# showlab/DiffSim

Hardware: AMD Instinct MI355X
Metric: image-pairs/sec at 512px, SD1.5 up_blocks[0] t=600 (higher is better)
Workload: dtype bf16

## Files before the change

### diffsim_amd/csrc/attention.hip

```cpp
#include "common.h"

#include <type_traits>

namespace dsim {
namespace {

__device__ __forceinline__ float max_halves(float x) {
    const unsigned u = __float_as_uint(x);
    const auto r = __builtin_amdgcn_permlane32_swap(u, u, false, false);
    return fmaxf(__uint_as_float(r[0]), __uint_as_float(r[1]));
}

constexpr int KT = 64;

template <typename T, int D> struct ACfg {
    static constexpr int ES = sizeof(T);
    static constexpr int VEC = 16 / ES;
    static constexpr int NKS = (D + 15) / 16;
    static constexpr int NDB = (D + 31) / 32;
    static constexpr int DPL = NDB * 32;
    static constexpr bool ONES = D < DPL;
    static constexpr int DPLK = (ES == 2) ? NKS * 16 : DPL;
    static constexpr int RS = DPLK * ES + 16;
    static constexpr bool KONE = (ES == 2) && (D % 16 == 8);
// ... 809 lines not shown
        if (__syncthreads_or(bad)) attend2<T, D, false>(qf, (const T*)p.k + kvoff, (const T*)p.v + kvoff, p.ldk, p.Nk, smem, oa, l);
    }
#pragma unroll
    for (int qb = 0; qb < 2; ++qb) {
        if (q[qb] >= p.Nq) continue;
        T* orow = (T*)p.out + ((size_t)b * p.Nq + q[qb]) * p.ldo + h * D;
        store_o_rows<D>(orow, half, wide_rows(p), [&](int db, int r) { return oa[qb].b[db][r]; });
    }
}

template <typename T, int D, bool FASTK>
__global__ __launch_bounds__(256, (ACfg<T, D>::WPS)) void attn_kernel(const AttnArgs p, const float scale_log2) {
    typedef ACfg<T, D> C;
    extern __shared__ __attribute__((aligned(16))) char smem[];
    const int lane = threadIdx.x & 63, wave = threadIdx.x >> 6, half = lane >> 5, l31 = lane & 31;
    const int nqb = (p.Nq + 127) / 128;
    int bid = blockIdx.x;
    if (p.xcd_remap) {
        const int nwg = gridDim.x, xcd = bid & 7, qq = nwg >> 3, r = nwg & 7, slot = bid >> 3;
        bid = (xcd < r ? xcd * (qq + 1) : r * (qq + 1) + (xcd - r) * qq) + slot;
    }
    const int qblk = bid % nqb, bh = bid / nqb;
    const int h = bh % p.H, b = bh / p.H;
    const int q = qblk * 128 + wave * 32 + l31;
    const int qc = q < p.Nq ? q : p.Nq - 1;
    const T* qrow = (const T*)p.q + ((size_t)b * p.Nq + qc) * p.ldq + h * D;
    QFrags<T, D> qf;
    load_q<T, D>(qf, qrow, half, scale_log2);
    const size_t kvoff = (size_t)(b % p.Bkv) * p.Nk * p.ldk + h * D;
    OAcc<T, D> oa;
    attend_checked<T, D, FASTK>(qf, (const T*)p.k + kvoff, (const T*)p.v + kvoff, p.ldk, p.Nk, smem, oa);
    auto& o = oa.b;
    if (q < p.Nq) {
        T* orow = (T*)p.out + ((size_t)b * p.Nq + q) * p.ldo + h * D;
        if constexpr (sizeof(T) == 2) {
            store_o_rows<D>((h16*)orow, half, wide_rows(p), [&](int db, int r) { return o[db][r]; });
        } else {
#pragma unroll
            for (int db = 0; db < C::NDB; ++db)
#pragma unroll
                for (int g = 0; g < 4; ++g) {
                    const int d = db * 32 + 8 * g + 4 * half;
                    if (d < D) {
                        f32x4 v4;
#pragma unroll
                        for (int j = 0; j < 4; ++j) v4[j] = o[db][4 * g + j];
                        *reinterpret_cast<f32x4*>(orow + d) = v4;
                    }
                }
        }
    }
}

template <int D, bool K80>
__global__ __launch_bounds__(256, 2) void attn_short_kernel(const AttnArgs p, const float scale_log2, const int qit) {
    typedef h16 T;
    typedef ACfg<T, D> C;
    constexpr int KR = 96;
    constexpr int CPRD = D / C::VEC;
    constexpr int VOFF = KR * C::RS;
    extern __shared__ __attribute__((aligned(16))) char smem[];
    const int tid = threadIdx.x, lane = tid & 63, wave = tid >> 6, half = lane >> 5, l31 = lane & 31;
    const int nqb = (p.Nq + 127) / 128;
    const int nbmax = (p.B + p.Bkv - 1) / p.Bkv;
    const int nch = (nbmax * nqb + qit - 1) / qit;
    int bid = blockIdx.x;
    if (p.xcd_remap) {
        const int nwg = gridDim.x, xcd = bid & 7, qq = nwg >> 3, r = nwg & 7, slot = bid >> 3;
        bid = (xcd < r ? xcd * (qq + 1) : r * (qq + 1) + (xcd - r) * qq) + slot;
    }
    const int h = bid % p.H, t0 = bid / p.H, ch = t0 % nch, bkv = t0 / nch;
    const int nbg = (p.B - bkv + p.Bkv - 1) / p.Bkv;
    if (ch * qit >= nbg * nqb) return;
    const size_t kvoff = (size_t)bkv * p.Nk * p.ldk + h * D;
    const T* kb = (const T*)p.k + kvoff;
    const T* vb = (const T*)p.v + kvoff;
    {
        const u32x4 z = {0u, 0u, 0u, 0u};
        for (int o = tid * 16; o < KR * (C::RS + C::RSV); o += 256 * 16) *reinterpret_cast<u32x4*>(smem + o) = z;
        __syncthreads();
        for (int idx = tid; idx < p.Nk * CPRD; idx += 256) {
            const int r = idx / CPRD, c = idx - r * CPRD;
            const u32x4 kk = *reinterpret_cast<const u32x4*>(kb + (size_t)r * p.ldk + c * C::VEC);
            const u32x4 vv = *reinterpret_cast<const u32x4*>(vb + (size_t)r * p.ldk + c * C::VEC);
            *reinterpret_cast<u32x4*>(smem + r * C::RS + c * 16) = kk;
            *reinterpret_cast<u32x4*>(smem + VOFF + r * C::RSV + c * 16) = vv;
        }
        if constexpr (C::ONES)
            for (int r = tid; r < p.Nk; r += 256) *reinterpret_cast<u32x4*>(smem + VOFF + r * C::RSV + CPRD * 16) = one_chunk<T>();
        __syncthreads();
    }
    const int i16 = lane & 15, g4 = lane >> 4;
    const char* const kfr = smem + l31 * C::RS + half * 16;
    const char* const vfr = smem + VOFF + (4 * (g4 >> 1) + (i16 >> 2)) * C::RSV + (16 * (g4 & 1) + 4 * (i16 & 3)) * 2;
    auto load_q_raw = [&](QFrags<T, D>& f, int b, int q) {
        const int qq = q < p.Nq ? q : p.Nq - 1;
        const T* qrow = (const T*)p.q + ((size_t)b * p.Nq + qq) * p.ldq + h * D;
#pragma unroll
        for (int ks = 0; ks < C::NKS; ++ks) {
            const int d0 = 16 * ks + 8 * half;
            if (d0 < D) f.f[ks] = *reinterpret_cast<const h16x8*>(qrow + d0);
            else zero_frag(f.f[ks]);
        }
    };
    float bias[8];
#pragma unroll
    for (int r = 0; r < 8; ++r) bias[r] = (64 + (r & 3) + 8 * (r >> 2) + 4 * half >= p.Nk) ? -INFINITY : 0.f;
    typedef float f32x2 __attribute__((ext_vector_type(2)));
    const f32x2 c2 = {scale_log2, scale_log2};
    const bool wide = wide_rows(p);

    int bi = (ch * qit) / nqb, qblk = ch * qit - bi * nqb;
    QFrags<T, D> qf;
    load_q_raw(qf, bi * p.Bkv + bkv, qblk * 128 + wave * 32 + l31);
    for (int it = 0; it < qit && bi < nbg; ++it) {
        const int b = bi * p.Bkv + bkv;
        const int q = qblk * 128 + wave * 32 + l31;
        if (++qblk == nqb) { qblk = 0; ++bi; }
        QFrags<T, D> qn;
        load_q_raw(qn, (bi < nbg ? bi : nbg - 1) * p.Bkv + bkv, qblk * 128 + wave * 32 + l31);
        if (q - l31 < p.Nq) {
            f32x16 s[3];
#pragma unroll
            for (int kbk = 0; kbk < 3; ++kbk) {
#pragma unroll
                for (int r = 0; r < 16; ++r) s[kbk][r] = 0.f;
#pragma unroll
                for (int ks = 0; ks < C::NKS; ++ks) {
                    h16x8 kf;
                    lload_frag(kf, kfr + kbk * 32 * C::RS + ks * 32);
                    mma(kf, qf.f[ks], s[kbk]);
                }
            }
            float m = -INFINITY;
#pragma unroll
            for (int kbk = 0; kbk < 3; ++kbk)
#pragma unroll
                for (int r = 0; r < ((K80 && kbk == 2) ? 8 : 16); ++r) {
                    if constexpr (!K80) {
                        const int kv = kbk * 32 + (r & 3) + 8 * (r >> 2) + 4 * half;
                        if (kv >= p.Nk) s[kbk][r] = -INFINITY;
                    } else if (kbk == 2) {
                        s[kbk][r] += bias[r];
                    }
                    m = fmaxf(m, s[kbk][r]);
                }
            m = max_halves(m);
            const float mc = -m * scale_log2;
            const f32x2 m2 = {mc, mc};
            float psum = 0.f;
#pragma unroll
            for (int kbk = 0; kbk < 3; ++kbk)
#pragma unroll
                for (int r = 0; r < ((K80 && kbk == 2) ? 8 : 16); r += 2) {
                    const f32x2 e = __builtin_elementwise_fma((f32x2){s[kbk][r], s[kbk][r + 1]}, c2, m2);
                    s[kbk][r] = __builtin_amdgcn_exp2f(e[0]);
                    s[kbk][r + 1] = __builtin_amdgcn_exp2f(e[1]);
                    if constexpr (!C::ONES) psum += s[kbk][r] + s[kbk][r + 1];
                }
            f32x16 o[C::NDB];
#pragma unroll
            for (int db = 0; db < C::NDB; ++db)
#pragma unroll
                for (int r = 0; r < 16; ++r) o[db][r] = 0.f;
#pragma unroll
            for (int kbk = 0; kbk < 3; ++kbk)
#pragma unroll
                for (int s2 = 0; s2 < ((K80 && kbk == 2) ? 1 : 2); ++s2) {
                    h16x8 pf;
#pragma unroll
                    for (int e = 0; e < 8; ++e) pf[e] = (h16)s[kbk][8 * s2 + e];
#pragma unroll
                    for (int db = 0; db < C::NDB; ++db) {
                        const char* pa = vfr + (kbk * 32 + 16 * s2) * C::RSV + db * 64;
                        const h16x4 lo = h16_ds_read_tr16_b64((pa));
                        const h16x4 hi = h16_ds_read_tr16_b64((pa + 8 * C::RSV));
                        h16x8 vf;
#pragma unroll
                        for (int e = 0; e < 4; ++e) { vf[e] = lo[e]; vf[4 + e] = hi[e]; }
                        o[db] = H16_MFMA_32x32x16(vf, pf, o[db], 0, 0, 0);
                    }
                }
            float l_tot;
            if constexpr (C::ONES) {
                constexpr int RB = D / 32, RR = D % 32;
                constexpr int RH = (RR >> 2) & 1, REG = (RR & 3) + 4 * (RR >> 3);
                const float mine = o[RB][REG];
                const float other = __shfl_xor(mine, 32);
                l_tot = (half == RH) ? mine : other;
            } else {
                l_tot = psum + __shfl_xor(psum, 32);
            }
            const float inv = 1.0f / l_tot;
            if (q < p.Nq) {
                T* orow = (T*)p.out + ((size_t)b * p.Nq + q) * p.ldo + h * D;
                store_o_rows<D>(orow, half, wide, [&](int db, int r) { return o[db][r] * inv; });
            }
        }
        qf = qn;
    }
}


template <typename T, int D, typename S, typename F>
__device__ __forceinline__ S fold_rounded(const OAcc<T, D>& acc, int half, S s, F&& f) {
    typedef float f32x2 __attribute__((ext_vector_type(2)));
#pragma unroll
    for (int db = 0; db < ACfg<T, D>::NDB; ++db)
#pragma unroll
        for (int r = 0; r < 16; r += 2) {
            T v[2];
            if constexpr (sizeof(T) == 2) {
                const h16x2 p = __builtin_convertvector((f32x2){acc.b[db][r], acc.b[db][r + 1]}, h16x2);
                v[0] = p[0]; v[1] = p[1];
            } else {
                v[0] = acc.b[db][r]; v[1] = acc.b[db][r + 1];
            }
#pragma unroll
            for (int e = 0; e < 2; ++e) {
                const int rr = r + e, d = db * 32 + (rr & 3) + 8 * (rr >> 2) + 4 * half;
                if (d < D) s = f(s, db, rr, d, v[e]);
            }
        }
    return s;
}

template <typename T, int D>
__device__ __forceinline__ void settle(OAcc<T, D>& acc) {
#pragma unroll
    for (int db = 0; db < ACfg<T, D>::NDB; ++db)
#pragma unroll
        for (int r = 0; r < 16; ++r) {
            if (db * 32 + (r & 3) + 8 * (r >> 2) >= D) continue;
            float x = acc.b[db][r];
            asm volatile("" : "+v"(x));
            acc.b[db][r] = x;
        }
}

struct TailSums { float s0 = 0.f, s1 = 0.f, s2 = 0.f; };
template <typename T, int D, typename Y>
__device__ __forceinline__ TailSums tail_products(const OAcc<T, D>& ox, int half, int mse, Y&& y) {
    return fold_rounded<T, D>(ox, half, TailSums{}, [&](TailSums s, int db, int r, int d, T xr) {
        const float x = (float)xr, yv = y(db, r, d);
        if (mse) { const float df = x - yv; s.s0 = fmaf(df, df, s.s0); }
        else { s.s0 = fmaf(x, yv, s.s0); s.s1 = fmaf(x, x, s.s1); s.s2 = fmaf(yv, yv, s.s2); }
        return s;
    });
}

__device__ __forceinline__ void store_block_partial(TailSums t, int lane, int wave, float* __restrict__ o) {
    __shared__ float red[4][4];
// ... 125 lines not shown
        set = (int)blockIdx.z >= p.n_a;
        iq = ix = (int)blockIdx.z - (set ? p.n_a : 0);
    } else {
        qtile = blockIdx.x % qt;
        const int cd = blockIdx.x / qt;
        cell = cd >> 1; dir = cd & 1;
        const int ia = cell / p.n_b, ib = cell - ia * p.n_b;
        set = dir;
        iq = dir ? ib : ia;
        ix = dir ? ia : ib;
    }
    const T* qg = (const T*)p.q[set];
    const T* kg = (const T*)p.k[set ^ (self_mode ? 0 : 1)];
    const T* vg = (const T*)p.v[set ^ (self_mode ? 0 : 1)];
    T* so = (T*)p.self[set] + iq * img + boff;
    const int q = qtile * 128 + wave * 32 + l31;
    const int qc = q < N ? q : N - 1;
    QFrags<T, D> qf;
    load_q<T, D>(qf, qg + iq * img + boff + (size_t)qc * ld, half, scale_log2);
    OAcc<T, D> oa;
    attend<T, D>(qf, kg + ix * img + boff, vg + ix * img + boff, ld, N, smem, oa);
    settle<T, D>(oa);
    if (self_mode) {
        if (q < N) fold_rounded<T, D>(oa, half, 0, [&](int, int, int, int d, T y) { so[(size_t)q * ld + d] = y; return 0; });
        return;
    }
    TailSums t;
    if (q < N) t = tail_products<T, D>(oa, half, mse, [&](int, int, int d) { return (float)so[(size_t)q * ld + d]; });
    store_block_partial(t, lane, wave, part + ((((size_t)cell * 2 + dir) * gridDim.y + bh) * qt + qtile) * 4);
}

inline float scale_log2_of(int D) { return (1.0f / sqrtf((float)D)) * 1.4426950408889634f; }


constexpr int ATTN_FAST_MIN = 1024;

AttnKernel attention_kernel(const AttnArgs& a, int dtype) {
    if (dtype == DSIM_F32) return AttnKernel::Exact;
    if (sdpa160_applies(a)) return AttnKernel::P160;
    if ((a.D == 40 || a.D == 64 || a.D == 80 || a.D == 160) && a.Nk <= 96)
        return a.Nk > 64 && a.Nk <= 80 ? AttnKernel::ShortK80 : AttnKernel::Short;
    if (a.D == 40 && a.Nk >= 2048 && a.Nk % KT == 0) return AttnKernel::Long;
    if (a.D == 64 && a.Nk > 96 && a.Nq >= 256) return a.Nk >= ATTN_FAST_MIN ? AttnKernel::Q2Fast : AttnKernel::Q2;
    return a.Nk >= ATTN_FAST_MIN ? AttnKernel::Fast : AttnKernel::Exact;
}

template <typename T, int D>
int launch_attn_d(const AttnArgs& a, AttnKernel kind, hipStream_t s) {
    typedef ACfg<T, D> C;
    switch (kind) {
        case AttnKernel::Short:
        case AttnKernel::ShortK80:
            if constexpr (sizeof(T) == 2 && (D == 40 || D == 64 || D == 80 || D == 160)) {
                constexpr int LDSK = 96 * (C::RS + C::RSV);
                constexpr int LDSS = LDSK < 56 * 1024 ? 56 * 1024 : LDSK;
                const int nqb = (a.Nq + 127) / 128, nvb = ((a.B + a.Bkv - 1) / a.Bkv) * nqb;
                const long want = (D > 80 ? 2L : 8L) * cu_count();
                int qit = 8;
                while (qit > 1 && (long)((nvb + qit - 1) / qit) * a.H * a.Bkv < want) qit >>= 1;
                const int nch = (nvb + qit - 1) / qit;
                const dim3 g(nch * a.H * a.Bkv);
                if (kind == AttnKernel::ShortK80) {
                    static DeviceOnce onces;
                    auto kern = attn_short_kernel<D, true>;
                    CK_ONCE(onces, kern, LDSS);
                    hipLaunchKernelGGL(kern, g, dim3(256), LDSS, s, a, scale_log2_of(D), qit);
                    g_attn_last_launch = AttnLaunchRec{DSIM_ATTN_SHORT_K80, D, DSIM_H16, 1, qit, (int)g.x};
                } else {
                    static DeviceOnce onces;
                    auto kern = attn_short_kernel<D, false>;
                    CK_ONCE(onces, kern, LDSS);
                    hipLaunchKernelGGL(kern, g, dim3(256), LDSS, s, a, scale_log2_of(D), qit);
                    g_attn_last_launch = AttnLaunchRec{DSIM_ATTN_SHORT, D, DSIM_H16, 0, qit, (int)g.x};
                }
                DSIM_HIP_CHECK(hipGetLastError());
                return DSIM_OK;
            }
            break;
        case AttnKernel::Long:
            if constexpr (sizeof(T) == 2 && D == 40) {
                constexpr int LDS3 = 3 * 2 * C::TILE;
#ifdef DSIM_DEVTOOLS
                switch (g_attn_dbg) {
#define X(d) case d: { static DeviceOnce o; auto k = attn_long_kernel<D, d>; CK_ONCE(o, k, LDS3); hipLaunchKernelGGL(k, dim3(((a.Nq + 255) / 256) * a.H * a.B), dim3(256), LDS3, s, a, scale_log2_of(D)); DSIM_HIP_CHECK(hipGetLastError()); return DSIM_OK; }
                    X(8) X(32) X(64) X(96)
#undef X
                    default: break;
                }
#endif
                static DeviceOnce once2;
                auto kern = attn_long_kernel<D, 0>;
                CK_ONCE(once2, kern, LDS3);
                const dim3 gl(((a.Nq + 255) / 256) * a.H * a.B);
                hipLaunchKernelGGL(kern, gl, dim3(256), LDS3, s, a, scale_log2_of(D));
                g_attn_last_launch = AttnLaunchRec{DSIM_ATTN_LONG, D, DSIM_H16, 0, 0, (int)gl.x};
                DSIM_HIP_CHECK(hipGetLastError());
                return DSIM_OK;
            }
            break;
        case AttnKernel::Q2:
        case AttnKernel::Q2Fast:
            if constexpr (sizeof(T) == 2 && D == 64) {
                const dim3 grid2(((a.Nq + 255) / 256) * a.H * a.B);
                if (kind == AttnKernel::Q2Fast) {
                    static DeviceOnce o1;
                    auto k = attn_q2_kernel<D, true>;
                    CK_ONCE(o1, k, C::LDS);
                    hipLaunchKernelGGL(k, grid2, dim3(256), C::LDS, s, a, scale_log2_of(D));
                    g_attn_last_launch = AttnLaunchRec{DSIM_ATTN_Q2FAST, D, DSIM_H16, 0, 0, (int)grid2.x};
                } else {
                    static DeviceOnce o2;
                    auto k = attn_q2_kernel<D, false>;
                    CK_ONCE(o2, k, C::LDS);
                    hipLaunchKernelGGL(k, grid2, dim3(256), C::LDS, s, a, scale_log2_of(D));
// ... 129 lines not shown
            }
        }
        red[1][t] = x2t; red[2][t] = y2t;
        __syncthreads();
        for (int s = NT / 2; s > 0; s >>= 1) {
            if (t < s) { red[1][t] += red[1][t + s]; red[2][t] += red[2][t + s]; }
            __syncthreads();
        }
        const double den = mse ? (double)BH * N * D : fmax(sqrt(red[1][0]), 1e-8) * fmax(sqrt(red[2][0]), 1e-8);
        double ct = 0.0;
        for (int i = t; i < N; i += NT) {
            const double c = fold(0, i) / den;
            ct += c;
            if (co) co[i] = (float)c;
        }
        __syncthreads();
        red[0][t] = ct;
        __syncthreads();
        for (int s = NT / 2; s > 0; s >>= 1) {
            if (t < s) red[0][t] += red[0][t + s];
            __syncthreads();
        }
        res += red[0][0];
        __syncthreads();
    }
    if (t == 0) {
        const float sc = (float)(res * 0.5);
        score[p] = sc;
        if (status) status[p] = (sc - sc == 0.0f) ? 0 : 1;
    }
}

template <typename T>
int launch_maps_t(const void* q, const void* k, const void* v, const int32_t* ia, const int32_t* ib, int n_pairs, int B, int H, int N,
                  int D, int mse, float* score, float* local, float* contrib, int32_t* status, void* scratch, hipStream_t s) {
    return with_head_dim(D, [&](auto dc) -> int {
        constexpr int Dc = decltype(dc)::value, LDS = ACfg<T, Dc>::LDS;
        static DeviceOnce once;
        auto kern = pair_map_kernel<T, Dc>;
        CK_ONCE(once, kern, LDS);
        hipLaunchKernelGGL(kern, dim3((N + 127) / 128, B * H, n_pairs * 2), dim3(256), LDS, s, (const T*)q, (const T*)k, (const T*)v, ia,
                           ib, B, H, N, scale_log2_of(Dc), mse, (float*)scratch);
        hipLaunchKernelGGL(pair_map_finish_kernel, dim3(n_pairs), dim3(MAP_FINISH_THREADS), 0, s, (const float*)scratch, B * H, N, Dc,
                           mse, score, local, contrib, status);
        DSIM_HIP_CHECK(hipGetLastError());
        return DSIM_OK;
    });
}

}

#ifdef DSIM_DEVTOOLS
int g_attn_dbg = 0;
#endif

inline namespace DSIM_H16_NS {
const char* attention_kernel_kind(const AttnArgs& a, int dtype) { return attn_kind_suffix((int)attention_kernel(a, dtype)); }

static bool attention_args_ok(const AttnArgs& a, int dtype) {
    const int vec = dtype == DSIM_F32 ? 4 : 8;
    return !(a.D % 8 || a.ldq % vec || a.ldk % vec || a.ldo % 4 || a.Nk < 1 || a.Nq < 1 || a.Bkv < 1);
}

int attention_plan(const AttnArgs& a, int dtype) {
    if (!attention_args_ok(a, dtype)) return DSIM_ERR_INVALID;
    bool own = dtype == DSIM_H16;
#ifndef DSIM_H16_IS_F16
    own |= dtype == DSIM_F32;
    if (dtype == DSIM_F16) return DSIM_F16_TWIN(attention_plan(a, dtype));
#endif
    if (!own) return DSIM_ERR_INVALID;
    const int st = with_head_dim(a.D, [](auto) { return DSIM_OK; });
    return st != DSIM_OK ? st : (int)attention_kernel(a, dtype);
}

int launch_attention(const AttnArgs& a, int dtype, hipStream_t s) {
    if (!attention_args_ok(a, dtype)) return DSIM_ERR_INVALID;
    if (dtype == DSIM_H16) {
        const AttnKernel kind = attention_kernel(a, dtype);
        return kind == AttnKernel::P160 ? launch_sdpa160(a, s) : launch_attn_t<h16>(a, kind, s);
    }
#ifndef DSIM_H16_IS_F16
    if (dtype == DSIM_F32) return launch_attn_t<float>(a, attention_kernel(a, dtype), s);
    if (dtype == DSIM_F16) return DSIM_F16_TWIN(launch_attention(a, dtype, s));
#endif
    return DSIM_ERR_INVALID;
}

size_t pair_score_scratch_bytes(int n_pairs, int B, int H, int N, int D) {
    const size_t tiled = (size_t)n_pairs * 2 * B * H * ((N + 127) / 128) * 4 * sizeof(float);
    if (pair_score160_applies(N, D, DSIM_H16)) {
        const size_t pers = pair_score160_scratch_bytes(n_pairs, B, H);
        return pers > tiled ? pers : tiled;
    }
    return tiled;
}

int launch_pair_score(const void* q, const void* k, const void* v, const int32_t* ia, const int32_t* ib,
                      int n_pairs, int B, int H, int N, int D, int dtype, int similarity, float* out, void* scratch,
                      size_t scratch_bytes, hipStream_t s, int32_t* status) {
    if (n_pairs <= 0 || D % 8 || N < 1) return DSIM_ERR_INVALID;
    if (scratch_bytes < pair_score_scratch_bytes(n_pairs, B, H, N, D)) return DSIM_ERR_WORKSPACE;
    if (n_pairs * 2 > 65535) return DSIM_ERR_INVALID;
    if (dtype == DSIM_H16) {
        if (pair_score160_applies(N, D, DSIM_H16))
            return launch_pair_score160(q, k, v, ia, ib, n_pairs, B, H, similarity, out, scratch, scratch_bytes, s, status);
// ... 67 lines not shown
```

### diffsim_amd/csrc/common.h

```cpp
#pragma once
#include <hip/hip_runtime.h>
#include <stddef.h>
#include <stdint.h>

#include "../../include/diffsim_amd.h"

namespace dsim {

typedef __bf16 bf16_t;
typedef _Float16 f16_t;
#ifdef DSIM_H16_IS_F16
typedef _Float16 h16;
#define DSIM_H16_NS f16
#define DSIM_H16 DSIM_F16
#define DSIM_H16_ONE_BITS 0x3C00u
#define DSIM_H16_LSUM_MAX 3.0e4f
#define H16_MFMA_16x16x32 __builtin_amdgcn_mfma_f32_16x16x32_f16
#define H16_MFMA_32x32x16 __builtin_amdgcn_mfma_f32_32x32x16_f16
#else
typedef __bf16 h16;
#define DSIM_H16_NS bf16
#define DSIM_H16 DSIM_BF16
#define DSIM_H16_ONE_BITS 0x3F80u
#define DSIM_H16_LSUM_MAX 1e30f
// ... 34 lines not shown

enum GemmMode { GEMM_LINEAR = 0, GEMM_CONV3 = 1, GEMM_CONV3P = 2 };
enum GemmEpi { EPI_NONE = 0, EPI_RESIDUAL = 1, EPI_GEGLU = 2 };

struct GemmArgs {
    const void* A0 = nullptr;
    const void* A1 = nullptr;
    int C0 = 0, C1 = 0;
    int mode = GEMM_LINEAR;
    int Hin = 0, Win = 0, Hout = 0, Wout = 0;
    int stride = 1, ups = 0;
    int pad = 1;
    int lwo = -1, lhw = -1;
    int M = 0, N = 0, K = 0;
    const void* W = nullptr;
    const float* bias = nullptr;
    const float* bias2 = nullptr;
    int rows_per_batch = 0;
    int act = 0;
    const float* gate = nullptr;
    const float* gate2 = nullptr;
    int epi = EPI_NONE;
    int geglu_blk = 32;
    const void* residual = nullptr;
    void* out = nullptr;
    int ldo = 0;
    int out_split = 0;
    long long out_split_stride = 0;
    int force_big = 0;
    int wb_rows = 0;
    unsigned wb_stride = 0;
    float* gn_part = nullptr;
    int gn_hw = 0;
    const void* zero_page = nullptr;
    unsigned a0_bytes = 0, a1_bytes = 0, w_bytes = 0, out_bytes = 0;
#ifdef DSIM_DEVTOOLS
    int exp = 0;
    unsigned long long* stamps = nullptr;
#endif
};
struct GemmLaunchRec {
    int bm = 0, bn = 0, mode = -1, geglu = 0, ek = -1, small = 0;
};
extern thread_local GemmLaunchRec g_gemm_last_launch;
inline int geglu_block_rows(int N) { return (N % 320 == 0 && N != 8 * 320) ? 16 : 32; }
#ifdef DSIM_DEVTOOLS
extern int g_gemm_persistent;
extern int g_force_bm;
extern int g_gemm_exp;
extern int g_gemm_skinny;
extern unsigned long long* g_gemm_stamps;
extern int g_skinny_tile;
extern int g_attn_dbg;
extern float* g_tail160_dbg;
extern int g_tail160_exp;
extern int g_ff_dbg;
extern int g_rl_dbg;
extern int g_rl_wpc;
extern int g_ff_stagger;
#else
constexpr int g_gemm_skinny = 1, g_gemm_persistent = 1, g_force_bm = 0;
#endif
int pack_linear(const void* src, int src_dtype, void* dst, int dst_dtype, int N, int K,
                int geglu_interleave, hipStream_t s);
int pack_conv3(const void* src, int src_dtype, void* dst, int dst_dtype, int Cout, int Cin,
               hipStream_t s);
int pack_conv_in(const void* src, int src_dtype, float* dst, int Cout, int Cin, hipStream_t s);
int pack_vector(const void* src, int src_dtype, float* dst, int N, int geglu_interleave,
                hipStream_t s);
int gemv_f32(const void* W, int w_dtype, const void* bias, int b_dtype, const float* x, float* y,
             int N, int K, int act, hipStream_t s);
int add_vectors_f32(const float* a, const float* b, float* out, int N, hipStream_t s);
int timestep_sincos(float* out, int dim, int t, hipStream_t s);
int sincos_values(float* out, int dim, const float* vals , int count, hipStream_t s);

int prep_conv_in(const float* lat, const float* noise , float sa, float sb, const float* w ,
                 const float* bias, void* out, int dtype, int n_img, int Cin, int S, int Cout, int dup ,
                 hipStream_t st);
bool conv_in_rows_applies(int Cin, int S, int Cout);
int conv_in_rows(const float* images, const float* w , const float* bias, void* out, int dtype, int n_img, int S,
                 float* gn_part, hipStream_t st);
int convert_f32_to(const float* src, void* dst, int dtype, size_t n, hipStream_t s);
int gather_ctx(const float* ctx, int n_ctx, const int32_t* index, void* dst, int dtype, int n_images, size_t per, hipStream_t s);
int dup_batch(const void* in, void* out, int n_batch, size_t bytes_per_elem, hipStream_t s);
int resize_nearest(const void* in, void* out, int B, int Hin, int Win, int Hout, int Wout, size_t row_bytes, hipStream_t s);

struct RowLinArgs {
    const void* x = nullptr;
    void* out = nullptr;
    const float* ln_g = nullptr;
    const float* ln_b = nullptr;
    const void* stream = nullptr;
    int M = 0, C = 0, N = 0;
    float eps = 1e-5f;
    int dtype = DSIM_BF16;
};

int image_preprocess(const unsigned char* hwc, float* out, int n, int H, int W, int half, hipStream_t s);
int latent_sample(const float* moments, const float* eps, float* out, int n_out, int first, int stride, int C, int hw, int eps_n,
                  float sf, int round16, hipStream_t s);

size_t groupnorm_scratch_bytes(int B, int groups);
int groupnorm_passes(int C0, int C1, int HW, int groups, int dtype);
int groupnorm_plan(int C0, int C1, int B, int HW, int groups, int dtype, int pre, dsim_gn_plan* plan);
int layernorm_plan(int M, int C, int dtype, int mod, dsim_ln_plan* plan);
int launch_groupnorm(const void* x0, int C0, const void* x1, int C1, const float* gamma,
// ... 102 lines not shown
```

### diffsim_amd/csrc/rowres.hip

```cpp
#include "common.h"

namespace dsim {
namespace {

constexpr int RC = 320;
constexpr int RKS = RC / 16;
constexpr int RNB = RC / 32;
constexpr int RNCH = 4 * RC / 32;
constexpr int RITER = RNCH + 2;
constexpr int RW1B = 64 * RC * 2;
constexpr int RW2B = RC * 64;
constexpr int RCHB = RW1B + RW2B;
constexpr int RPIECES = RCHB / 1024;
constexpr int RPW = RPIECES / 4;
constexpr int RB1 = 0, RB2 = 8 * RC, RLG = 9 * RC, RLB = 10 * RC, RVEC = 11 * RC;
constexpr int RSCR = 32 * 144;
constexpr int RLDS = 2 * RCHB + RVEC * 4 + 4 * RSCR;
static_assert(RPIECES % 4 == 0 && RITER % 2 == 0, "ring geometry");

__global__ void pack_ff_stream_kernel(const h16* __restrict__ w1p, const h16* __restrict__ w2p, char* __restrict__ stream) {
    const int i = blockIdx.x * blockDim.x + threadIdx.x;
    if (i >= RITER * (RCHB / 16)) return;
    const int ci = i / (RCHB / 16), o = (i - ci * (RCHB / 16)) * 16;
    u32x4 v = {0u, 0u, 0u, 0u};
// ... 20 lines not shown
}

struct FFParams {
    const h16* x;
    h16* out;
    const float* ln_g;
    const float* ln_b;
    const char* stream;
    const float* b1;
    const float* b2;
    int M;
    float eps;
    unsigned x_bytes, stream_bytes;
    int stagger;
};

template <int DBG>
__global__ __launch_bounds__(256, 1) void ff_fused_kernel(const FFParams p, const int ntiles) {
    extern __shared__ __attribute__((aligned(16))) char smem[];
    const int tid = threadIdx.x, lane = tid & 63, l31 = lane & 31, half = lane >> 5;
    const int wave = __builtin_amdgcn_readfirstlane(tid >> 6);
    constexpr unsigned OOB = 0x80000000u;

    const __amdgpu_buffer_rsrc_t rX = __builtin_amdgcn_make_buffer_rsrc((void*)p.x, 0, (int)p.x_bytes, 0x00020000);
    const __amdgpu_buffer_rsrc_t rO = __builtin_amdgcn_make_buffer_rsrc((void*)p.out, 0, (int)p.x_bytes, 0x00020000);
    const __amdgpu_buffer_rsrc_t rS = __builtin_amdgcn_make_buffer_rsrc((void*)p.stream, 0, (int)p.stream_bytes, 0x00020000);

    auto dma = [&](int sp, int ci, int d) {
        if (DBG & 1) return;
        char* dst = smem + sp * RCHB + wave * (RPW * 1024) + d * 1024;
        __builtin_amdgcn_raw_ptr_buffer_load_lds(rS, (__attribute__((address_space(3))) void*)dst, 16, lane * 16,
                                                 ci * RCHB + wave * (RPW * 1024) + d * 1024, 0, 0);
    };
#pragma unroll
    for (int d = 0; d < RPW; ++d) dma(0, 0, d);
    float* const vec = reinterpret_cast<float*>(smem + 2 * RCHB);
    for (int i = tid; i < RVEC / 4; i += 256) {
        const int e = 4 * i;
        const float* src = e < RB2 ? p.b1 + e : (e < RLG ? p.b2 + (e - RB2) : (e < RLB ? p.ln_g + (e - RLG) : p.ln_b + (e - RLB)));
        *reinterpret_cast<f32x4*>(vec + e) = *reinterpret_cast<const f32x4*>(src);
    }

    const int sw1 = (l31 >> 1) & 7;
    int w1off[4];
#pragma unroll
    for (int kk = 0; kk < 4; ++kk) w1off[kk] = l31 * 128 + (((2 * kk + half) ^ sw1) << 4);
    const int sw2 = (l31 >> 2) & 3;
    int w2off[2];
#pragma unroll
    for (int s = 0; s < 2; ++s) w2off[s] = RW1B + l31 * 64 + (((2 * s + half) ^ sw2) << 4);

    u32x4 raw[RKS];
    auto load_rows = [&](int tile) {
        const int row = tile * 128 + wave * 32 + l31;
        const unsigned rbase = (tile < ntiles && row < p.M) ? (unsigned)row * (RC * 2) + half * 16 : OOB;
#pragma unroll
        for (int ks = 0; ks < RKS; ++ks) raw[ks] = __builtin_amdgcn_raw_buffer_load_b128(rX, (int)(rbase + ks * 32), 0, 0);
    };
    load_rows(blockIdx.x);
    __syncthreads();

    for (int tile = blockIdx.x; tile < ntiles; tile += gridDim.x) {
        const int m0 = tile * 128 + wave * 32;
        h16x8 X[RKS];
        {
            float sum = 0.f;
#pragma unroll
            for (int ks = 0; ks < RKS; ++ks) {
                const h16x8 t = __builtin_bit_cast(h16x8, raw[ks]);
#pragma unroll
                for (int j = 0; j < 8; ++j) sum += (float)t[j];
            }
            {
                const unsigned u = __float_as_uint(sum);
                const auto r = __builtin_amdgcn_permlane32_swap(u, u, false, false);
                sum = __uint_as_float(r[0]) + __uint_as_float(r[1]);
            }
            const float mean = sum * (1.0f / RC);
            float sq = 0.f;
#pragma unroll
            for (int ks = 0; ks < RKS; ++ks) {
                asm volatile("" : "+v"(raw[ks]));
                const h16x8 t = __builtin_bit_cast(h16x8, raw[ks]);
#pragma unroll
                for (int j = 0; j < 8; ++j) { const float d = (float)t[j] - mean; sq = fmaf(d, d, sq); }
            }
            {
                const unsigned u = __float_as_uint(sq);
                const auto r = __builtin_amdgcn_permlane32_swap(u, u, false, false);
                sq = __uint_as_float(r[0]) + __uint_as_float(r[1]);
            }
            const float rstd = 1.0f / sqrtf(sq * (1.0f / RC) + p.eps);
#pragma unroll
            for (int ks = 0; ks < RKS; ++ks) {
                const int c = 16 * ks + 8 * half;
                const f32x4 g0 = *reinterpret_cast<const f32x4*>(vec + RLG + c), g1 = *reinterpret_cast<const f32x4*>(vec + RLG + c + 4);
                const f32x4 b0 = *reinterpret_cast<const f32x4*>(vec + RLB + c), b1 = *reinterpret_cast<const f32x4*>(vec + RLB + c + 4);
                asm volatile("" : "+v"(raw[ks]));
                const h16x8 t = __builtin_bit_cast(h16x8, raw[ks]);
#pragma unroll
                for (int j = 0; j < 4; ++j) {
                    X[ks][j] = (h16)fmaf(((float)t[j] - mean) * rstd, g0[j], b0[j]);
                    X[ks][4 + j] = (h16)fmaf(((float)t[4 + j] - mean) * rstd, g1[j], b1[j]);
                }
            }
        }
        __builtin_amdgcn_sched_barrier(0);
        f32x16 out[RNB];
#pragma unroll
        for (int b = 0; b < RNB; ++b)
#pragma unroll
            for (int q = 0; q < 4; ++q) {
                const f32x4 b4 = *reinterpret_cast<const f32x4*>(vec + RB2 + 32 * b + 8 * q + 4 * half);
#pragma unroll
                for (int e = 0; e < 4; ++e) out[b][4 * q + e] = b4[e];
            }
// ... 149 lines not shown
    const int i = blockIdx.x * blockDim.x + threadIdx.x;
    if (i >= N / 32 * (LCHB / 16)) return;
    const int b = i / (LCHB / 16), o = (i - b * (LCHB / 16)) * 16;
    const int slab = o / 4096, row = (o % 4096) / 128, cpos = (o % 128) / 16;
    const int cl = cpos ^ ((row >> 1) & 7);
    *reinterpret_cast<u32x4*>(stream + (size_t)b * LCHB + o) =
        *reinterpret_cast<const u32x4*>(wp + (size_t)(32 * b + row) * RC + 64 * slab + 8 * cl);
}

struct RLParams {
    const h16* x;
    h16* out;
    const float* ln_g;
    const float* ln_b;
    const char* stream;
    int M, N;
    float eps;
    unsigned x_bytes, out_bytes, stream_bytes;
};

template <int DBG>
__global__ __launch_bounds__(256, 3) void rowlin_kernel(const RLParams p, const int ntiles) {
    extern __shared__ __attribute__((aligned(16))) char smem[];
    const int tid = threadIdx.x, lane = tid & 63, l31 = lane & 31, half = lane >> 5;
    const int wave = __builtin_amdgcn_readfirstlane(tid >> 6);
    constexpr unsigned OOB = 0x80000000u;
    const __amdgpu_buffer_rsrc_t rX = __builtin_amdgcn_make_buffer_rsrc((void*)p.x, 0, (int)p.x_bytes, 0x00020000);
    const __amdgpu_buffer_rsrc_t rO = __builtin_amdgcn_make_buffer_rsrc((void*)p.out, 0, (int)p.out_bytes, 0x00020000);
    const __amdgpu_buffer_rsrc_t rS = __builtin_amdgcn_make_buffer_rsrc((void*)p.stream, 0, (int)p.stream_bytes, 0x00020000);
    const int nblk = p.N / 32;
    auto dma = [&](int sp, int blk) {
        char* dst = smem + sp * LCHB + wave * (LPW * 1024);
#pragma unroll
        for (int d = 0; d < LPW; ++d)
            __builtin_amdgcn_raw_ptr_buffer_load_lds(rS, (__attribute__((address_space(3))) void*)(dst + d * 1024), 16, lane * 16,
                                                     blk * LCHB + wave * (LPW * 1024) + d * 1024, 0, 0);
    };
    dma(0, 0);
    float* const vec = reinterpret_cast<float*>(smem + 2 * LCHB);
    if (p.ln_g)
        for (int i = tid; i < LVEC; i += 256) vec[i] = i < RC ? p.ln_g[i] : p.ln_b[i - RC];
    char* const slab = smem + 2 * LCHB + LVEC * 4 + wave * LSCR;
    const int sw1 = (l31 >> 1) & 7;
    int woff[4];
#pragma unroll
    for (int kk = 0; kk < 4; ++kk) woff[kk] = l31 * 128 + (((2 * kk + half) ^ sw1) << 4);
    __syncthreads();
    int blk = 0;

    for (int tile = blockIdx.x; tile < ntiles; tile += gridDim.x) {
        const int m0 = tile * 128 + wave * 32;
        u32x4 xr[RKS];
        {
            const int row = m0 + l31;
            const unsigned rbase = row < p.M ? (unsigned)row * (RC * 2) + half * 16 : OOB;
#pragma unroll
            for (int ks = 0; ks < RKS; ++ks)
                xr[ks] = (DBG & 4) ? u32x4{(unsigned)ks, 1u, 2u, rbase} : __builtin_amdgcn_raw_buffer_load_b128(rX, (int)(rbase + ks * 32), 0, 0);
            if (p.ln_g) {
                float sum = 0.f;
#pragma unroll
                for (int ks = 0; ks < RKS; ++ks) {
                    const h16x8 t = __builtin_bit_cast(h16x8, xr[ks]);
#pragma unroll
                    for (int j = 0; j < 8; ++j) sum += (float)t[j];
                }
                {
                    const unsigned u = __float_as_uint(sum);
                    const auto r = __builtin_amdgcn_permlane32_swap(u, u, false, false);
                    sum = __uint_as_float(r[0]) + __uint_as_float(r[1]);
                }
                const float mean = sum * (1.0f / RC);
                float sq = 0.f;
#pragma unroll
                for (int ks = 0; ks < RKS; ++ks) {
                    asm volatile("" : "+v"(xr[ks]));
                    const h16x8 t = __builtin_bit_cast(h16x8, xr[ks]);
#pragma unroll
                    for (int j = 0; j < 8; ++j) { const float d = (float)t[j] - mean; sq = fmaf(d, d, sq); }
                }
                {
                    const unsigned u = __float_as_uint(sq);
                    const auto r = __builtin_amdgcn_permlane32_swap(u, u, false, false);
                    sq = __uint_as_float(r[0]) + __uint_as_float(r[1]);
                }
                const float rstd = 1.0f / sqrtf(sq * (1.0f / RC) + p.eps);
#pragma unroll
                for (int ks = 0; ks < RKS; ++ks) {
                    const int c = 16 * ks + 8 * half;
                    const f32x4 g0 = *reinterpret_cast<const f32x4*>(vec + c), g1 = *reinterpret_cast<const f32x4*>(vec + c + 4);
                    const f32x4 b0 = *reinterpret_cast<const f32x4*>(vec + RC + c), b1 = *reinterpret_cast<const f32x4*>(vec + RC + c + 4);
                    asm volatile("" : "+v"(xr[ks]));
                    const h16x8 t = __builtin_bit_cast(h16x8, xr[ks]);
                    h16x8 y;
#pragma unroll
                    for (int j = 0; j < 4; ++j) {
                        y[j] = (h16)fmaf(((float)t[j] - mean) * rstd, g0[j], b0[j]);
                        y[4 + j] = (h16)fmaf(((float)t[4 + j] - mean) * rstd, g1[j], b1[j]);
                    }
                    xr[ks] = __builtin_bit_cast(u32x4, y);
                    __builtin_amdgcn_sched_barrier(0);
                }
            }
        }
        __builtin_amdgcn_sched_barrier(0);
        h16x8 wf[2][2];
        auto step = [&](int sp, f32x16& a) {
            if (sp == 0) asm volatile("s_waitcnt vmcnt(4)" ::: "memory");
            else asm volatile("s_waitcnt vmcnt(0)" ::: "memory");
            __syncthreads();
            const int nb = blk + 1 == nblk ? 0 : blk + 1;
// ... 43 lines not shown
                    const u32x4 t = *reinterpret_cast<const u32x4*>(slab + r * 144 + c * 16);
                    if (!(DBG & 1) || t[0] == 0x12345u) __builtin_amdgcn_raw_buffer_store_b128(t, rO, (int)go, 0, 0);
                }
            }
        };
        f32x16 a0, a1;
        for (int pr = 0; pr < nblk / 2; ++pr) {
            step(0, a0);
            step(1, a1);
            store_pair(a0, a1, 64 * pr);
        }
    }
    asm volatile("s_waitcnt vmcnt(0)" ::: "memory");
}

}

#ifdef DSIM_DEVTOOLS
int g_rl_dbg = 0;
int g_ff_dbg = 0;
int g_ff_stagger = -1;
int g_rl_wpc = 3;
#endif

inline namespace DSIM_H16_NS {
size_t ff_stream_bytes(int C) { return C == RC ? (size_t)RITER * RCHB : 0; }

int pack_ff_stream(const void* w1_packed, const void* w2_packed, void* stream, int C, hipStream_t s) {
    if (C != RC) return DSIM_ERR_INVALID;
    const int n = RITER * (RCHB / 16);
    hipLaunchKernelGGL(pack_ff_stream_kernel, dim3((n + 255) / 256), dim3(256), 0, s, (const h16*)w1_packed,
                       (const h16*)w2_packed, (char*)stream);
    DSIM_HIP_CHECK(hipGetLastError());
    return DSIM_OK;
}

int launch_ff_fused(const FFArgs& a, hipStream_t s) {
    if (a.dtype != DSIM_H16) return a.dtype == DSIM_F16 ? DSIM_F16_TWIN(launch_ff_fused(a, s)) : DSIM_ERR_INVALID;
    if (a.C != RC || a.M < 1 || (size_t)a.M * RC * 2 >= 0x7fffffffull) return DSIM_ERR_INVALID;
    FFParams p;
    p.x = (const h16*)a.x; p.out = (h16*)a.out; p.ln_g = a.ln_g; p.ln_b = a.ln_b; p.stream = (const char*)a.stream;
    p.b1 = a.b1; p.b2 = a.b2; p.M = a.M; p.eps = a.eps;
    p.x_bytes = (unsigned)((size_t)a.M * RC * 2);
    p.stream_bytes = (unsigned)((size_t)RITER * RCHB);
    p.stagger = 1;
#ifdef DSIM_DEVTOOLS
    if (g_ff_stagger >= 0) p.stagger = g_ff_stagger;
#endif
    const int ntiles = (a.M + 127) / 128;
    const int grid = ntiles < cu_count() ? ntiles : cu_count();
#ifdef DSIM_DEVTOOLS
    switch (g_ff_dbg) {
#define X(d) case d: { static DeviceOnce o; auto k = ff_fused_kernel<d>; CK_ONCE(o, k, RLDS); hipLaunchKernelGGL(k, dim3(grid), dim3(256), RLDS, s, p, ntiles); DSIM_HIP_CHECK(hipGetLastError()); return DSIM_OK; }
        X(1) X(2) X(3) X(12) X(13) X(15) X(16) X(31)
#undef X
        default: break;
    }
#endif
    static DeviceOnce once;
    auto kern = ff_fused_kernel<0>;
    CK_ONCE(once, kern, RLDS);
    hipLaunchKernelGGL(kern, dim3(grid), dim3(256), RLDS, s, p, ntiles);
    DSIM_HIP_CHECK(hipGetLastError());
    return DSIM_OK;
}

size_t rowlin_stream_bytes(int C, int N) { return (C == RC && N % 64 == 0 && N <= 960) ? (size_t)N / 32 * LCHB : 0; }

int pack_rowlin_stream(const void* w_packed, void* stream, int C, int N, hipStream_t s) {
    if (!rowlin_stream_bytes(C, N)) return DSIM_ERR_INVALID;
    const int n = N / 32 * (LCHB / 16);
    hipLaunchKernelGGL(pack_rowlin_stream_kernel, dim3((n + 255) / 256), dim3(256), 0, s, (const h16*)w_packed, (char*)stream, N);
    DSIM_HIP_CHECK(hipGetLastError());
    return DSIM_OK;
}

int launch_rowlin(const RowLinArgs& a, hipStream_t s) {
    if (a.dtype != DSIM_H16) return a.dtype == DSIM_F16 ? DSIM_F16_TWIN(launch_rowlin(a, s)) : DSIM_ERR_INVALID;
    if (!rowlin_stream_bytes(a.C, a.N) || a.M < 1 || (size_t)a.M * a.N * 2 >= 0x7fffffffull || !a.ln_g != !a.ln_b) return DSIM_ERR_INVALID;
    RLParams p;
    p.x = (const h16*)a.x; p.out = (h16*)a.out; p.ln_g = a.ln_g; p.ln_b = a.ln_b; p.stream = (const char*)a.stream;
    p.M = a.M; p.N = a.N; p.eps = a.eps;
    p.x_bytes = (unsigned)((size_t)a.M * RC * 2); p.out_bytes = (unsigned)((size_t)a.M * a.N * 2);
    p.stream_bytes = (unsigned)rowlin_stream_bytes(a.C, a.N);
    const int ntiles = (a.M + 127) / 128;
#ifdef DSIM_DEVTOOLS
    const int wpc = g_rl_wpc;
#else
    constexpr int wpc = 3;
#endif
    const int grid = ntiles < wpc * cu_count() ? ntiles : wpc * cu_count();
#ifdef DSIM_DEVTOOLS
    switch (g_rl_dbg) {
#define X(d) case d: { static DeviceOnce o; auto k = rowlin_kernel<d>; CK_ONCE(o, k, LLDS); hipLaunchKernelGGL(k, dim3(grid), dim3(256), LLDS, s, p, ntiles); DSIM_HIP_CHECK(hipGetLastError()); return DSIM_OK; }
        X(1) X(2) X(4) X(8) X(10) X(15)
#undef X
        default: break;
    }
#endif
    static DeviceOnce once;
    auto kern = rowlin_kernel<0>;
    CK_ONCE(once, kern, LLDS);
    hipLaunchKernelGGL(kern, dim3(grid), dim3(256), LLDS, s, p, ntiles);
    DSIM_HIP_CHECK(hipGetLastError());
    return DSIM_OK;
}
}

}
```

Baseline: 674.4.

## Stage Q loads and O stores through per-wave LDS slab for coalesced access

For head dims up to 80, the short-key attention kernel now loads Q as contiguous 16-byte chunks spread across lanes, transposes them through a per-wave LDS slab into MFMA fragment layout, and stages the normalized output the same way before writing full rows. The goal is coalesced global reads and writes in place of the per-lane strided row accesses. It costs extra LDS space (kept within the two-workgroups-per-CU budget) and adds LDS round trips. Ablation switches and coalesced-load debug variants for the rowres kernels are added behind devtools flags.

```diff
diff --git a/diffsim_amd/csrc/attention.hip b/diffsim_amd/csrc/attention.hip
--- a/diffsim_amd/csrc/attention.hip
+++ b/diffsim_amd/csrc/attention.hip
@@ -885,10 +885,19 @@
     }
 }
 
-template <int D, bool K80>
+template <int D> struct ShortIO {
+    static constexpr int CPRD = D / 8;
+    static constexpr bool SLAB = D <= 80;
+    static constexpr int SS = (CPRD | 1) * 16;
+    static constexpr int NCH = (32 * CPRD + 63) / 64;
+    static constexpr int BYTES = SLAB ? 4 * 32 * SS : 0;
+};
+template <int D, bool K80, int ABL = 0>
 __global__ __launch_bounds__(256, 2) void attn_short_kernel(const AttnArgs p, const float scale_log2, const int qit) {
     typedef h16 T;
     typedef ACfg<T, D> C;
+    typedef ShortIO<D> IO;
+    constexpr bool SLAB = IO::SLAB && !(ABL & 1);
     constexpr int KR = 96;
     constexpr int CPRD = D / C::VEC;
     constexpr int VOFF = KR * C::RS;
@@ -932,9 +941,37 @@
 #pragma unroll
         for (int ks = 0; ks < C::NKS; ++ks) {
             const int d0 = 16 * ks + 8 * half;
-            if (d0 < D) f.f[ks] = *reinterpret_cast<const h16x8*>(qrow + d0);
+            if ((ABL & 2) && d0 < D) f.f[ks] = __builtin_bit_cast(h16x8, u32x4{(unsigned)q, 0u, 0u, (unsigned)ks});
+            else if (d0 < D) f.f[ks] = *reinterpret_cast<const h16x8*>(qrow + d0);
             else zero_frag(f.f[ks]);
         }
+    };
+    struct QChunks { u32x4 c[IO::NCH]; };
+    char* const slab = smem + KR * (C::RS + C::RSV) + wave * (32 * IO::SS);
+    int crow[IO::NCH], ccol[IO::NCH];
+#pragma unroll
+    for (int i = 0; i < IO::NCH; ++i) { const int g = 64 * i + lane; crow[i] = g / CPRD; ccol[i] = g - crow[i] * CPRD; }
+    auto load_q_chunks = [&](QChunks& f, int b, int q0) {
+#pragma unroll
+        for (int i = 0; i < IO::NCH; ++i) {
+            if (64 * i + lane >= 32 * CPRD) continue;
+            const int q = q0 + crow[i], qq = q < p.Nq ? q : p.Nq - 1;
+            const T* src = (const T*)p.q + ((size_t)b * p.Nq + qq) * p.ldq + h * D + 8 * ccol[i];
+            f.c[i] = (ABL & 2) ? u32x4{(unsigned)q, 0u, 0u, (unsigned)i} : *reinterpret_cast<const u32x4*>(src);
+        }
+    };
+    auto chunks_to_frags = [&](const QChunks& f, QFrags<T, D>& o) {
+        asm volatile("" ::: "memory");
+#pragma unroll
+        for (int i = 0; i < IO::NCH; ++i)
+            if (64 * i + lane < 32 * CPRD) *reinterpret_cast<u32x4*>(slab + crow[i] * IO::SS + ccol[i] * 16) = f.c[i];
+        asm volatile("" ::: "memory");
+#pragma unroll
+        for (int ks = 0; ks < C::NKS; ++ks) {
+            if (16 * ks + 8 * half < D) o.f[ks] = *reinterpret_cast<const h16x8*>(slab + l31 * IO::SS + (2 * ks + half) * 16);
+            else zero_frag(o.f[ks]);
+        }
+        asm volatile("" ::: "memory");
     };
     float bias[8];
 #pragma unroll
@@ -945,13 +982,17 @@
 
     int bi = (ch * qit) / nqb, qblk = ch * qit - bi * nqb;
     QFrags<T, D> qf;
-    load_q_raw(qf, bi * p.Bkv + bkv, qblk * 128 + wave * 32 + l31);
+    QChunks qc;
+    if constexpr (SLAB) load_q_chunks(qc, bi * p.Bkv + bkv, qblk * 128 + wave * 32);
+    else load_q_raw(qf, bi * p.Bkv + bkv, qblk * 128 + wave * 32 + l31);
     for (int it = 0; it < qit && bi < nbg; ++it) {
         const int b = bi * p.Bkv + bkv;
         const int q = qblk * 128 + wave * 32 + l31;
         if (++qblk == nqb) { qblk = 0; ++bi; }
+        if constexpr (SLAB) chunks_to_frags(qc, qf);
         QFrags<T, D> qn;
-        load_q_raw(qn, (bi < nbg ? bi : nbg - 1) * p.Bkv + bkv, qblk * 128 + wave * 32 + l31);
+        if constexpr (SLAB) load_q_chunks(qc, (bi < nbg ? bi : nbg - 1) * p.Bkv + bkv, qblk * 128 + wave * 32);
+        else load_q_raw(qn, (bi < nbg ? bi : nbg - 1) * p.Bkv + bkv, qblk * 128 + wave * 32 + l31);
         if (q - l31 < p.Nq) {
             f32x16 s[3];
 #pragma unroll
@@ -1025,12 +1066,36 @@
                 l_tot = psum + __shfl_xor(psum, 32);
             }
             const float inv = 1.0f / l_tot;
-            if (q < p.Nq) {
+            if (SLAB && wide) {
+                asm volatile("" ::: "memory");
+#pragma unroll
+                for (int db = 0; db < C::NDB; ++db)
+#pragma unroll
+                    for (int g = 0; g < 4; ++g) {
+                        const int d = db * 32 + 8 * g + 4 * half;
+                        if (d < D) {
+                            const h16x2 v0 = __builtin_convertvector((f32x2){o[db][4 * g] * inv, o[db][4 * g + 1] * inv}, h16x2);
+                            const h16x2 v1 = __builtin_convertvector((f32x2){o[db][4 * g + 2] * inv, o[db][4 * g + 3] * inv}, h16x2);
+                            *reinterpret_cast<u32x2*>(slab + l31 * IO::SS + d * 2) = u32x2{__builtin_bit_cast(unsigned, v0), __builtin_bit_cast(unsigned, v1)};
+                        }
+                    }
+                asm volatile("" ::: "memory");
+#pragma unroll
+                for (int i = 0; i < IO::NCH; ++i) {
+                    const int qo = q - l31 + crow[i];
+                    if (64 * i + lane < 32 * CPRD && qo < p.Nq) {
+                        const u32x4 t = *reinterpret_cast<const u32x4*>(slab + crow[i] * IO::SS + ccol[i] * 16);
+                        if (!(ABL & 4) || t[0] == 0x12345u)
+                            *reinterpret_cast<u32x4*>((T*)p.out + ((size_t)b * p.Nq + qo) * p.ldo + h * D + 8 * ccol[i]) = t;
+                    }
+                }
+                asm volatile("" ::: "memory");
+            } else if (q < p.Nq) {
                 T* orow = (T*)p.out + ((size_t)b * p.Nq + q) * p.ldo + h * D;
-                store_o_rows<D>(orow, half, wide, [&](int db, int r) { return o[db][r] * inv; });
-            }
-        }
-        qf = qn;
+                if (!(ABL & 4) || inv == 0.12345f) store_o_rows<D>(orow, half, wide, [&](int db, int r) { return o[db][r] * inv; });
+            }
+        }
+        if constexpr (!SLAB) qf = qn;
     }
 }
 
@@ -1262,14 +1327,26 @@
         case AttnKernel::Short:
         case AttnKernel::ShortK80:
             if constexpr (sizeof(T) == 2 && (D == 40 || D == 64 || D == 80 || D == 160)) {
-                constexpr int LDSK = 96 * (C::RS + C::RSV);
+                constexpr int LDSK = 96 * (C::RS + C::RSV) + ShortIO<D>::BYTES;
                 constexpr int LDSS = LDSK < 56 * 1024 ? 56 * 1024 : LDSK;
+                static_assert(LDSS <= 80 * 1024 || D > 80, "two workgroups per CU");
                 const int nqb = (a.Nq + 127) / 128, nvb = ((a.B + a.Bkv - 1) / a.Bkv) * nqb;
                 const long want = (D > 80 ? 2L : 8L) * cu_count();
                 int qit = 8;
                 while (qit > 1 && (long)((nvb + qit - 1) / qit) * a.H * a.Bkv < want) qit >>= 1;
                 const int nch = (nvb + qit - 1) / qit;
                 const dim3 g(nch * a.H * a.Bkv);
+#ifdef DSIM_DEVTOOLS
+                switch (g_short_abl) {
+#define X(m) case m: { static DeviceOnce o0, o1; auto k0 = attn_short_kernel<D, false, m>; auto k1 = attn_short_kernel<D, true, m>; \
+                       if (kind == AttnKernel::ShortK80) { CK_ONCE(o1, k1, LDSS); hipLaunchKernelGGL(k1, g, dim3(256), LDSS, s, a, scale_log2_of(D), qit); } \
+                       else { CK_ONCE(o0, k0, LDSS); hipLaunchKernelGGL(k0, g, dim3(256), LDSS, s, a, scale_log2_of(D), qit); } \
+                       DSIM_HIP_CHECK(hipGetLastError()); return DSIM_OK; }
+                    X(1) X(2) X(4) X(6) X(3) X(5) X(7)
+#undef X
+                    default: break;
+                }
+#endif
                 if (kind == AttnKernel::ShortK80) {
                     static DeviceOnce onces;
                     auto kern = attn_short_kernel<D, true>;
@@ -1505,6 +1582,7 @@
 
 #ifdef DSIM_DEVTOOLS
 int g_attn_dbg = 0;
+int g_short_abl = 0;
 #endif
 
 inline namespace DSIM_H16_NS {
diff --git a/diffsim_amd/csrc/common.h b/diffsim_amd/csrc/common.h
--- a/diffsim_amd/csrc/common.h
+++ b/diffsim_amd/csrc/common.h
@@ -110,6 +110,7 @@
 extern unsigned long long* g_gemm_stamps;
 extern int g_skinny_tile;
 extern int g_attn_dbg;
+extern int g_short_abl;
 extern float* g_tail160_dbg;
 extern int g_tail160_exp;
 extern int g_ff_dbg;
diff --git a/diffsim_amd/csrc/rowres.hip b/diffsim_amd/csrc/rowres.hip
--- a/diffsim_amd/csrc/rowres.hip
+++ b/diffsim_amd/csrc/rowres.hip
@@ -96,6 +96,15 @@
 
     u32x4 raw[RKS];
     auto load_rows = [&](int tile) {
+        if (DBG & 32) {
+#pragma unroll
+            for (int i = 0; i < RKS; ++i) {
+                const int idx = lane + (i & 3) * 64, row = tile * 128 + wave * 32 + (idx >> 3);
+                const unsigned go = (tile < ntiles && row < p.M) ? (unsigned)row * (RC * 2) + (unsigned)((i >> 2) * 128 + (idx & 7) * 16) : OOB;
+                raw[i] = __builtin_amdgcn_raw_buffer_load_b128(rX, (int)go, 0, 0);
+            }
+            return;
+        }
         const int row = tile * 128 + wave * 32 + l31;
         const unsigned rbase = (tile < ntiles && row < p.M) ? (unsigned)row * (RC * 2) + half * 16 : OOB;
 #pragma unroll
@@ -106,6 +115,22 @@
 
     for (int tile = blockIdx.x; tile < ntiles; tile += gridDim.x) {
         const int m0 = tile * 128 + wave * 32;
+        if (DBG & 32) {
+            char* const slab = smem + 2 * RCHB + RVEC * 4 + wave * RSCR;
+#pragma unroll
+            for (int g = 0; g < RKS / 4; ++g) {
+                asm volatile("" ::: "memory");
+#pragma unroll
+                for (int it = 0; it < 4; ++it) {
+                    const int idx = lane + it * 64;
+                    *reinterpret_cast<u32x4*>(slab + (idx >> 3) * 144 + (idx & 7) * 16) = raw[4 * g + it];
+                }
+                asm volatile("" ::: "memory");
+#pragma unroll
+                for (int kk = 0; kk < 4; ++kk) raw[4 * g + kk] = *reinterpret_cast<const u32x4*>(slab + l31 * 144 + (2 * kk + half) * 16);
+            }
+            asm volatile("" ::: "memory");
+        }
         h16x8 X[RKS];
         {
             float sum = 0.f;
@@ -361,11 +386,41 @@
         const int m0 = tile * 128 + wave * 32;
         u32x4 xr[RKS];
         {
-            const int row = m0 + l31;
-            const unsigned rbase = row < p.M ? (unsigned)row * (RC * 2) + half * 16 : OOB;
-#pragma unroll
-            for (int ks = 0; ks < RKS; ++ks)
-                xr[ks] = (DBG & 4) ? u32x4{(unsigned)ks, 1u, 2u, rbase} : __builtin_amdgcn_raw_buffer_load_b128(rX, (int)(rbase + ks * 32), 0, 0);
+            if (!(DBG & 16)) {
+                const int row = m0 + l31;
+                const unsigned rbase = row < p.M ? (unsigned)row * (RC * 2) + half * 16 : OOB;
+#pragma unroll
+                for (int ks = 0; ks < RKS; ++ks)
+                    xr[ks] = (DBG & 4) ? u32x4{(unsigned)ks, 1u, 2u, rbase} : __builtin_amdgcn_raw_buffer_load_b128(rX, (int)(rbase + ks * 32), 0, 0);
+            } else {
+                u32x4 ld[RKS];
+#pragma unroll
+                for (int g = 0; g < RKS / 4; ++g)
+#pragma unroll
+                    for (int pi = 0; pi < 4; ++pi) {
+                        const int idx = lane + (pi & 1) * 64, r = idx >> 3, c = idx & 7, row = m0 + 16 * (pi >> 1) + r;
+                        const unsigned go = row < p.M ? (unsigned)row * (RC * 2) + (unsigned)(g * 128 + c * 16) : OOB;
+                        ld[4 * g + pi] = (DBG & 4) ? u32x4{(unsigned)g, 1u, 2u, go} : __builtin_amdgcn_raw_buffer_load_b128(rX, (int)go, 0, 0);
+                    }
+#pragma unroll
+                for (int g = 0; g < RKS / 4; ++g)
+#pragma unroll
+                    for (int ph = 0; ph < 2; ++ph) {
+                        asm volatile("" ::: "memory");
+#pragma unroll
+                        for (int it = 0; it < 2; ++it) {
+                            const int idx = lane + it * 64, r = idx >> 3, c = idx & 7;
+                            *reinterpret_cast<u32x4*>(slab + r * 144 + c * 16) = ld[4 * g + 2 * ph + it];
+                        }
+                        asm volatile("" ::: "memory");
+                        if (ph == 0 || l31 >= 16) {
+#pragma unroll
+                            for (int kk = 0; kk < 4; ++kk)
+                                xr[4 * g + kk] = *reinterpret_cast<const u32x4*>(slab + (l31 & 15) * 144 + (2 * kk + half) * 16);
+                        }
+                    }
+                asm volatile("" ::: "memory");
+            }
             if (p.ln_g) {
                 float sum = 0.f;
 #pragma unroll
@@ -515,7 +570,7 @@
 #ifdef DSIM_DEVTOOLS
     switch (g_ff_dbg) {
 #define X(d) case d: { static DeviceOnce o; auto k = ff_fused_kernel<d>; CK_ONCE(o, k, RLDS); hipLaunchKernelGGL(k, dim3(grid), dim3(256), RLDS, s, p, ntiles); DSIM_HIP_CHECK(hipGetLastError()); return DSIM_OK; }
-        X(1) X(2) X(3) X(12) X(13) X(15) X(16) X(31)
+        X(1) X(2) X(3) X(12) X(13) X(15) X(16) X(31) X(32)
 #undef X
         default: break;
     }
@@ -556,7 +611,7 @@
 #ifdef DSIM_DEVTOOLS
     switch (g_rl_dbg) {
 #define X(d) case d: { static DeviceOnce o; auto k = rowlin_kernel<d>; CK_ONCE(o, k, LLDS); hipLaunchKernelGGL(k, dim3(grid), dim3(256), LLDS, s, p, ntiles); DSIM_HIP_CHECK(hipGetLastError()); return DSIM_OK; }
-        X(1) X(2) X(4) X(8) X(10) X(15)
+        X(1) X(2) X(4) X(8) X(10) X(15) X(16) X(20)
 #undef X
         default: break;
     }
```

Result: no change. 674.1 (-0.0%).
